# dog-qiuqiu/Yolo-FastestV2

Hardware: NVIDIA H100
Metric: images/sec 352x352 fwd+decode+NMS (higher is better)
Workload: dtype f32

## Files before the change

include/yfv2.h:

```cpp
#ifndef YFV2_H_
#define YFV2_H_

#include <stddef.h>
#include <stdint.h>

#ifdef __cplusplus
extern "C" {
#endif

#define YFV2_OK            0
#define YFV2_EINVAL       -1
#define YFV2_ECUDA        -2
#define YFV2_EUNSUPPORTED -3
#define YFV2_ENOMEM       -4

#define YFV2_ABI_VERSION   1

#if defined(__GNUC__)
#define YFV2_API __attribute__((visibility("default")))
#else
#define YFV2_API
#endif

#define YFV2_NUM_PARAMS    225
// ... 34 lines not shown
YFV2_API int yfv2_nms_workspace_bytes(int N, int M, int C, size_t* bytes);
YFV2_API int yfv2_nms(const float* dets, int N, int M, int C, float conf_thres, double iou_thres,
             const int* class_filter, int n_filter, int max_det, float max_wh,
             float* out, int* counts, int* kept_idx, void* workspace, void* stream);

YFV2_API int yfv2_decode_nms(const float* const preds[6], int N, int H, int W, int A, int C,
                    const double* anchors_host, float conf_thres, double iou_thres,
                    const int* class_filter, int n_filter, int max_det, float max_wh,
                    float* out, int* counts, int* kept_idx, void* workspace, void* stream);

YFV2_API int yfv2_batch_statistics(const float* dets, const int* counts, int N, int max_det, const float* targets, int nt,
                                   float iou_threshold, float* tp, void* stream);

YFV2_API int yfv2_aug_contrast_brightness(const uint8_t* img, uint8_t* out, const float* alpha, const float* beta, int N,
                                          long long bytes_per_image, void* stream);

typedef struct yfv2_frame {
    const uint8_t* data;
    int w, h;
    long long pitch;
} yfv2_frame;
YFV2_API int yfv2_resize_bgr_u8(const yfv2_frame* frames, int N, int H, int W, uint8_t* dst, void* stream);

typedef struct yfv2_yuv420_frame {
    const uint8_t* y;
    long long y_pitch;
    const uint8_t* u;
    const uint8_t* v;
    long long uv_pitch;
    int uv_step;
    int w, h;
} yfv2_yuv420_frame;
YFV2_API int yfv2_resize_yuv420_u8(const yfv2_yuv420_frame* frames, int N, int H, int W, uint8_t* dst, void* stream);

YFV2_API int yfv2_detect_u8_host(yfv2_plan* plan, const uint8_t* x_host, const void* packed,
                        const double* anchors_host, float conf_thres, double iou_thres, int max_det,
                        float* out_host, int* counts_host, void* workspace, void* stream);
YFV2_API size_t yfv2_detect_workspace_bytes(const yfv2_plan* plan, int max_det);

YFV2_API int yfv2_loss_workspace_bytes(int N, int H, int W, int A, int C, int nt, size_t* bytes);
YFV2_API int yfv2_compute_loss(const float* const preds[6], const float* targets, int nt, int N, int H, int W, int A, int C,
                               const double* anchors_host, float* losses, float* const dpreds[6], void* workspace,
                               void* stream);
YFV2_API int yfv2_loss_read_targets(const void* workspace, int level, int N, int H, int W, int A, int nt, int* count_host,
                                    int* idx, float* tbox, double* anch, int* tcls, void* stream);

YFV2_API int yfv2_op_conv1x1_fwd(const float* x, const float* w, const float* bias, float* y, int N, int K, int M, int HW, void* stream);
YFV2_API int yfv2_op_conv1x1_bwd(const float* x, const float* w, const float* dy, float* dx, float* dw, float* dbias, int N, int K, int M,
                                 int HW, void* stream);
YFV2_API int yfv2_op_dwconv_fwd(const float* x, const float* w, float* y, int N, int C, int H, int W, int ks, int stride, void* stream);
YFV2_API int yfv2_op_dwconv_bwd(const float* x, const float* w, const float* dy, float* dx, float* dw, int N, int C, int H, int W, int ks,
                                int stride, void* stream);
YFV2_API int yfv2_op_stem_fwd(const float* x, const float* w, float* y, int N, int M, int H, int W, void* stream);
YFV2_API int yfv2_op_stem_wgrad(const float* x, const float* dy, float* dw, int N, int M, int H, int W, void* stream);
YFV2_API int yfv2_op_bn_train_fwd(const float* x, const float* gamma, const float* beta, float* running_mean, float* running_var, float* y,
                                  float* save_mean, float* save_invstd, double* scratch, int N, int C, int HW, int relu, void* stream);
YFV2_API int yfv2_op_bn_train_bwd(const float* x, const float* y, const float* dy, const float* gamma, const float* save_mean,
                                  const float* save_invstd, float* dx, float* dgamma, float* dbeta, double* scratch, int N, int C, int HW,
                                  int relu, void* stream);
YFV2_API int yfv2_op_maxpool_fwd(const float* x, float* y, int* idx, int planes, int H, int W, void* stream);
YFV2_API int yfv2_op_maxpool_bwd(const float* dy, const int* idx, float* dx, int planes, int H, int W, void* stream);
YFV2_API int yfv2_op_upsample2_fwd(const float* x, float* y, int planes, int H, int W, void* stream);
YFV2_API int yfv2_op_upsample2_bwd(const float* dy, float* dx, int planes, int H, int W, void* stream);

typedef struct yfv2_trainer yfv2_trainer;
YFV2_API int yfv2_trainer_create(yfv2_trainer** out, int device, int N, int H, int W, int A, int C);
YFV2_API void yfv2_trainer_destroy(yfv2_trainer* t);
YFV2_API int yfv2_trainer_workspace_bytes(const yfv2_trainer* t, size_t* bytes);
YFV2_API int yfv2_trainer_grad_floats(const yfv2_trainer* t, long long* n);
YFV2_API int yfv2_trainer_param_offset(const yfv2_trainer* t, int index, long long* offset, long long* numel);
YFV2_API int yfv2_train_forward(yfv2_trainer* t, const float* x, const float* const* params, float* const* bn_running,
                                float* const preds[6], void* workspace, void* stream);
YFV2_API int yfv2_train_backward(yfv2_trainer* t, const float* x, const float* const* params, float* const preds[6],
                                 const float* const dpreds[6], float* grads_flat, int accumulate, void* workspace, void* stream);

YFV2_API const char* yfv2_plan_stage_name(const yfv2_plan* plan, int i);
YFV2_API int yfv2_plan_stage_group(const yfv2_plan* plan, int i);
YFV2_API int yfv2_forward_range(yfv2_plan* plan, const void* x, int is_u8, const void* packed, float* const preds[6],
                                void* workspace, int first, int last, void* stream);

YFV2_API int yfv2_debug_gather(const yfv2_plan* plan, const void* workspace, int which, float* out, int* dims4,
                               void* stream);

YFV2_API int yfv2_debug_pw_tc(const float* x, const float* w, float* out, float* pack_ws, int K, int N, int P,
                              void* stream);

YFV2_API int yfv2_debug_nms_profile(long long* dev_buf);

#ifdef __cplusplus
}
#endif
#endif
```

yolo-fastestv2_b200/csrc/k_net.cu:

```cuda
#include "common.cuh"
#include "tc.cuh"

namespace yfv2 {

namespace {
using namespace tc;

constexpr int kThreads = 256;
constexpr int kWarps = kThreads / 32;
constexpr int kMaxChain = 7;
constexpr size_t kChainBudget = 110 * 1024;
constexpr size_t kBandBudget = 110 * 1024;

__host__ __device__ constexpr int pw_smem_floats(int K, int NP) { return K * w_stride(NP) + 2 * NP; }

__device__ void load_pw(float* dst, const float* __restrict__ src, int K, int N, int NP) {
    const int S = w_stride(NP), Np = round4(N);
    for (int i = threadIdx.x; i < K * NP; i += blockDim.x) {
        const int k = i / NP, n = i - k * NP;
        dst[k * S + n] = n < N ? __ldg(src + k * Np + n) : 0.f;
    }
    for (int n = threadIdx.x; n < NP; n += blockDim.x) {
        dst[K * S + n] = n < N ? __ldg(src + K * Np + n) : 0.f;
        dst[K * S + NP + n] = n < N ? __ldg(src + K * Np + Np + n) : 0.f;
// ... 659 lines not shown

template <int K>
int dispatch_blk(int stride, BlkArgs& a, int N, cudaStream_t s) {
    return stride == 1 ? run_blk<K, 1>(a, N, s) : run_blk<K, 2>(a, N, s);
}

template <class Kern>
int run_whole_image(Kern kern, size_t bytes, BlkArgs& a, int N, cudaStream_t s) {
    a.R = a.Ho; a.bands = 1; a.items = N;
    if (int rc = smem_attr(kern, bytes)) return rc;
    int per_sm = 0;
    YFV2_CUDA(cudaOccupancyMaxActiveBlocksPerMultiprocessor(&per_sm, kern, kThreads, bytes));
    YFV2_CUDA(launch_k(kern, persistent_grid(N, per_sm > 0 ? per_sm : 1), kThreads, bytes, s, pdl_take(), a));
    YFV2_LAUNCH_CHECK();
    return YFV2_OK;
}

struct FpnArgs {
    Planes c3, c2, out;
    unsigned short t3[192], t2[96];
    const float* pw;
    int N, H, W, chunks;
};

template <int KIN>
__global__ void __launch_bounds__(kThreads)
fpn_kernel(const __grid_constant__ FpnArgs p) {
    pdl_trigger();
    constexpr int NT = 9, S = w_stride(72);
    extern __shared__ __align__(16) float smem[];
    load_pw(smem, p.pw, KIN, 72, 72);
    pdl_wait();
    __syncthreads();
    const int warp = threadIdx.x >> 5, lane = threadIdx.x & 31, g = lane >> 2, t = lane & 3;
    const int HW = p.H * p.W;
    for (int item = blockIdx.x; item < p.N * p.chunks; item += gridDim.x) {
        const int n = item / p.chunks, m0 = (item - n * p.chunks) * 16 * kWarps + 16 * warp;
        if (m0 >= HW) continue;
        int o3[2], o2[2], oo[2]; bool ok[2];
#pragma unroll
        for (int h = 0; h < 2; ++h) {
            const int m = m0 + g + 8 * h, y = m / p.W, x = m - y * p.W;
            ok[h] = m < HW;
            const int yy = ok[h] ? y : 0, xx = ok[h] ? x : 0;
            o3[h] = KIN == 192 ? p.c3.org + yy * p.c3.Ws + xx : p.c3.org + (yy >> 1) * p.c3.Ws + (xx >> 1);
            o2[h] = p.c2.org + yy * p.c2.Ws + xx;
            oo[h] = p.out.org + yy * p.out.Ws + xx;
        }
        const float* b3 = p.c3.base + (long long)n * p.c3.sN;
        const float* b2 = p.c2.base + (long long)n * p.c2.sN;
        float acc[NT][4];
        warp_gemm<KIN / 8, NT>(acc, smem, S, [&](int ks, float (&a)[4]) {
#pragma unroll
            for (int q = 0; q < 2; ++q) {
                const int k = 8 * ks + t + 4 * q;
                const float* pl = k < 192 ? b3 + (long long)p.t3[k] * p.c3.sC : b2 + (long long)p.t2[k - 192] * p.c2.sC;
#pragma unroll
                for (int h = 0; h < 2; ++h) a[2 * q + h] = pl[k < 192 ? o3[h] : o2[h]];
            }
        });
        float* ob = p.out.base + (long long)n * p.out.sN;
        const float* sc = smem + KIN * S;
#pragma unroll
        for (int h = 0; h < 2; ++h) {
            if (!ok[h]) continue;
#pragma unroll
            for (int nt = 0; nt < NT; ++nt)
#pragma unroll
                for (int e = 0; e < 2; ++e) {
                    const int col = 8 * nt + 2 * t + e;
                    ob[(long long)col * p.out.sC + oo[h]] = fmaxf(fmaf(acc[nt][2 * h + e], sc[col], sc[72 + col]), 0.f);
                }
        }
    }
}

struct HeadArgs {
    Planes in[2], out[2];
    const float* dw[2];
    const float* pw[2];
    float* dst[2][2];
    int split[2], rowsA[2], rowsB[2];
    int N, H, W, chunks;
};

constexpr int kHeadTile = 96;

template <int HALF>
__device__ __forceinline__ void head_body(const HeadArgs& p) {
    pdl_trigger();
    constexpr int NP = HALF == 0 ? 72 : HALF == 1 ? kHeadTile : 2 * kHeadTile;
    constexpr int NT = HALF == 0 ? 9 : HALF == 1 ? kHeadTile / 8 : kHeadTile / 16, S = w_stride(NP);
    extern __shared__ __align__(16) float smem[];
    float* sW = smem;
    float* sD = sW + pw_smem_floats(72, NP);
    const int br = blockIdx.y;
    const int tiles = HALF == 2 && br == 0 ? 2 : 1;
    if (HALF == 0) {
        load_pw(sW, p.pw[br], 72, 72, 72);
    } else {
        const float* F = p.pw[br];
        const int NF = HALF == 2 ? kHeadTile * tiles : NP;
        for (int i = threadIdx.x; i < 72 * NF; i += kThreads) {
            const int k = i / NF, nn = i - k * NF;
            sW[k * S + nn] = __ldg(F + nn * 72 + k);
        }
        for (int nn = threadIdx.x; nn < NF; nn += kThreads) { sW[72 * S + nn] = 1.f; sW[72 * S + NP + nn] = __ldg(F + NF * 72 + nn); }
    }
    load_floats(sD, p.dw[br], 72 * 28);
    pdl_wait();
    __syncthreads();
    const int warp = threadIdx.x >> 5, lane = threadIdx.x & 31, g = lane >> 2, t = lane & 3;
    const int HW = p.H * p.W;
    const Planes in = p.in[br];
    for (int item = blockIdx.x; item < p.N * p.chunks; item += gridDim.x) {
        const int n = item / p.chunks, m0 = (item - n * p.chunks) * 16 * kWarps + 16 * warp;
        if (m0 >= HW) continue;
        int off[2]; bool ok[2];
#pragma unroll
        for (int h = 0; h < 2; ++h) {
            const int m = m0 + g + 8 * h, y = m / p.W, x = m - y * p.W;
            ok[h] = m < HW;
            off[h] = ok[h] ? in.org + (y - 2) * in.Ws + x - 2 : in.org;
        }
        const float* ib = in.base + (long long)n * in.sN;
        auto load_a = [&](int ks, float (&a)[4]) {
#pragma unroll
            for (int q = 0; q < 2; ++q) {
                const int k = 8 * ks + t + 4 * q;
                const float* w = sD + 28 * k;
                const float* pk = ib + (long long)k * in.sC;
#pragma unroll
                for (int h = 0; h < 2; ++h) {
                    const float* tp = pk + off[h];
                    float v = 0.f;
#pragma unroll
                    for (int dy = 0; dy < 5; ++dy)
#pragma unroll
                        for (int dx = 0; dx < 5; ++dx) v = fmaf(tp[dy * in.Ws + dx], w[dy * 5 + dx], v);
                    a[2 * q + h] = ok[h] ? fmaxf(fmaf(v, w[25], w[26]), 0.f) : 0.f;
                }
            }
        };
        auto store = [&](const float (&acc)[NT][4], int c0) {
            const float* sc = sW + 72 * S;
#pragma unroll
            for (int h = 0; h < 2; ++h) {
                if (!ok[h]) continue;
                const int m = m0 + g + 8 * h;
#pragma unroll
                for (int nt = 0; nt < NT; ++nt)
#pragma unroll
                    for (int e = 0; e < 2; ++e) {
                        const int col = c0 + 8 * nt + 2 * t + e;
                        const float v = fmaf(acc[nt][2 * h + e], sc[col], sc[NP + col]);
                        if (HALF == 0) {
                            const Planes& o = p.out[br];
                            const int y = m / p.W, x = m - y * p.W;
                            o.base[(long long)n * o.sN + (long long)col * o.sC + o.org + y * o.Ws + x] = v;
                        } else if (col < p.split[br]) {
                            p.dst[br][0][((long long)n * p.rowsA[br] + col) * HW + m] = v;
                        } else if (col < p.split[br] + p.rowsB[br]) {
                            p.dst[br][1][((long long)n * p.rowsB[br] + col - p.split[br]) * HW + m] = v;
                        }
                    }
            }
        };
        if constexpr (HALF < 2) {
            float acc[NT][4];
            warp_gemm<9, NT>(acc, sW, S, load_a);
            store(acc, 0);
        } else {
            float af[9][4];
#pragma unroll
            for (int ks = 0; ks < 9; ++ks) load_a(ks, af[ks]);
#pragma unroll 1
            for (int c0 = 0; c0 < kHeadTile * tiles; c0 += 8 * NT) {
                float acc[NT][4];
                warp_gemm_regs<9, NT>(acc, sW + c0, S, af);
                store(acc, c0);
            }
        }
    }
}

template <int HALF>
__global__ void __launch_bounds__(kThreads)
head_kernel(const __grid_constant__ HeadArgs p) { head_body<HALF>(p); }

__global__ void __launch_bounds__(kThreads, 2)
head2_kernel(const __grid_constant__ HeadArgs p) { head_body<2>(p); }

template <int K, int NP>
__global__ void __launch_bounds__(kThreads)
pw_test_kernel(const float* __restrict__ x, const float* __restrict__ w, float* __restrict__ out, int N, int P) {
    constexpr int S = w_stride(NP);
    extern __shared__ __align__(16) float smem[];
    for (int i = threadIdx.x; i < K * NP; i += kThreads) {
        const int k = i / NP, nn = i - k * NP;
        smem[k * S + nn] = nn < N ? w[nn * K + k] : 0.f;
    }
    __syncthreads();
    const int warp = threadIdx.x >> 5, lane = threadIdx.x & 31, g = lane >> 2, t = lane & 3;
    const int m0 = (blockIdx.x * kWarps + warp) * 16;
    if (m0 >= P) return;
    float acc[NP / 8][4];
    warp_gemm<K / 8, NP / 8>(acc, smem, S, [&](int ks, float (&a)[4]) {
#pragma unroll
        for (int q = 0; q < 2; ++q)
#pragma unroll
            for (int h = 0; h < 2; ++h) {
                const int m = m0 + g + 8 * h;
                a[2 * q + h] = m < P ? x[(size_t)(8 * ks + t + 4 * q) * P + m] : 0.f;
            }
    });
#pragma unroll
    for (int h = 0; h < 2; ++h) {
        const int m = m0 + g + 8 * h;
        if (m >= P) continue;
#pragma unroll
        for (int nt = 0; nt < NP / 8; ++nt)
#pragma unroll
            for (int e = 0; e < 2; ++e) {
                const int col = 8 * nt + 2 * t + e;
                if (col < N) out[(size_t)col * P + m] = acc[nt][2 * h + e];
            }
    }
}

template <int K, int NP>
int run_pw_test(const float* x, const float* w, float* out, int N, int P, cudaStream_t s) {
    const size_t bytes = (size_t)K * w_stride(NP) * sizeof(float);
    if (int rc = smem_attr(pw_test_kernel<K, NP>, bytes)) return rc;
    pw_test_kernel<K, NP><<<(P + 16 * kWarps - 1) / (16 * kWarps), kThreads, bytes, s>>>(x, w, out, N, P);
    YFV2_LAUNCH_CHECK();
    return YFV2_OK;
}

}

bool blk_s1_chainable(int K, int H, int W) {
    const size_t bytes = blk_smem_bytes(K, 1, H, W);
    return bytes <= kChainBudget || (K == 96 && bytes <= kSmemCap);
}

int blk_launch_s1(int K, const Planes& P, int nblk, const ChanTab* tin, const ChanTab* tout, const float* const* w1,
                  const float* const* wdw, const float* const* w2, int N, cudaStream_t s) {
    if (nblk < 1 || nblk > kMaxChain || (nblk > 1 && !blk_s1_chainable(K, P.H, P.W))) {
        set_error("block: a chain of %d stride-1 blocks needs a whole %dx%d image per CTA", nblk, P.H, P.W);
        return YFV2_EINVAL;
    }
    BlkArgs a{};
    a.in = P; a.out = P;
    a.Hi = a.Ho = P.H; a.Wi = a.Wo = P.W;
    a.nblk = nblk;
    a.R = nblk > 1 ? P.H : blk_rows(K, 1, P.H, P.W, N);
    for (int j = 0; j < nblk; ++j) {
        a.pw1[j] = w1[j]; a.dw[j] = wdw[j]; a.pw2[j] = w2[j];
        for (int i = 0; i < K; ++i) { a.tin[j][i] = tin[j].c[i]; a.tout[j][i] = tout[j].c[i]; }
    }
    const size_t bytes = blk_smem_bytes(K, 1, P.H, P.W);
    if (nblk > 1 && bytes > kChainBudget) return run_whole_image(blk_chain_kernel<96>, bytes, a, N, s);
    switch (K) {
    case 24: return dispatch_blk<24>(1, a, N, s);
    case 48: return dispatch_blk<48>(1, a, N, s);
    case 96: return dispatch_blk<96>(1, a, N, s);
    }
    set_error("block: unsupported width %d", K);
    return YFV2_EUNSUPPORTED;
}

int blk_launch_s2(int K, const Planes& in, const Planes& out, const ChanTab& tin, const ChanTab& tout, const float* wdwp, const float* wp,
                  const float* w1, const float* wdwm, const float* w2, int N, cudaStream_t s) {
    BlkArgs a{};
    a.in = in; a.out = out;
    a.Hi = in.H; a.Wi = in.W; a.Ho = out.H; a.Wo = out.W;
    a.nblk = 1;
    a.pw1[0] = w1; a.dw[0] = wdwm; a.pw2[0] = w2; a.dwp = wdwp; a.pwp = wp;
    for (int i = 0; i < K; ++i) { a.tin[0][i] = tin.c[i]; a.tout[0][i] = tout.c[i]; a.tmain[i] = tout.c[K + i]; }
    if (blk_s2_whole_image(K, out.H, out.W, in.W))
        return run_whole_image(blk_s2_image_kernel<96>, blk_s2_image_smem_bytes(K, out.H, in.W), a, N, s);
    a.R = blk_rows(K, 2, out.H, in.W, N);
    if (blk_s2_walk_fits(K, in)) return K == 24 ? run_blk_walk<24>(a, N, s) : run_blk_walk<48>(a, N, s);
    switch (K) {
    case 24: return dispatch_blk<24>(2, a, N, s);
    case 48: return dispatch_blk<48>(2, a, N, s);
    case 96: return dispatch_blk<96>(2, a, N, s);
    }
    set_error("block: unsupported width %d", K);
    return YFV2_EUNSUPPORTED;
}

int fpn_launch(int which, const Planes& c3, const ChanTab& t3, const Planes& c2, const ChanTab& t2, const Planes& out, const float* pw,
               int N, cudaStream_t s) {
    FpnArgs a{};
    a.c3 = c3; a.c2 = c2; a.out = out; a.pw = pw;
    for (int i = 0; i < 192; ++i) a.t3[i] = t3.c[i];
    for (int i = 0; i < 96; ++i) a.t2[i] = t2.c[i];
    a.N = N; a.H = out.H; a.W = out.W;
    a.chunks = (out.H * out.W + 16 * kWarps - 1) / (16 * kWarps);
    auto run = [&](auto kern, int kin) -> int {
        const size_t bytes = (size_t)pw_smem_floats(kin, 72) * sizeof(float);
        if (int rc = smem_attr(kern, bytes)) return rc;
        YFV2_CUDA(launch_k(kern, persistent_grid((long long)N * a.chunks, 2), kThreads, bytes, s, pdl_take(), a));
        YFV2_LAUNCH_CHECK();
        return YFV2_OK;
    };
    return which == 1 ? run(fpn_kernel<192>, 192) : run(fpn_kernel<288>, 288);
}

int heads_launch(int half, const Planes& sIn, const Planes& tcls, const Planes& treg, const float* const wdw[2], const float* const wpw[2],
                 float* reg, float* obj, float* cls, int A, int C, int N, cudaStream_t s) {
    HeadArgs a{};
    for (int b = 0; b < 2; ++b) { a.dw[b] = wdw[b]; a.pw[b] = wpw[b]; }
    a.out[0] = tcls; a.out[1] = treg;
    if (half == 0) { a.in[0] = sIn; a.in[1] = sIn; }
    else { a.in[0] = tcls; a.in[1] = treg; }
    a.dst[0][0] = obj; a.dst[0][1] = cls; a.split[0] = A; a.rowsA[0] = A; a.rowsB[0] = C;
    a.dst[1][0] = reg; a.dst[1][1] = reg; a.split[1] = 4 * A; a.rowsA[1] = 4 * A; a.rowsB[1] = 0;
    a.N = N; a.H = sIn.H; a.W = sIn.W;
    a.chunks = (sIn.H * sIn.W + 16 * kWarps - 1) / (16 * kWarps);
    auto run = [&](auto kern, int np) -> int {
        const size_t bytes = ((size_t)pw_smem_floats(72, np) + 72 * 28) * sizeof(float);
        if (int rc = smem_attr(kern, bytes)) return rc;
        cudaLaunchConfig_t cfg{};
        cfg.gridDim = dim3((unsigned)persistent_grid((long long)N * a.chunks, 1), 2);
        cfg.blockDim = dim3(kThreads); cfg.dynamicSmemBytes = bytes; cfg.stream = s;
        cudaLaunchAttribute at[1];
        at[0].id = cudaLaunchAttributeProgrammaticStreamSerialization;
        at[0].val.programmaticStreamSerializationAllowed = 1;
        cfg.attrs = at; cfg.numAttrs = pdl_take() ? 1 : 0;
        YFV2_CUDA(cudaLaunchKernelEx(&cfg, kern, a));
        YFV2_LAUNCH_CHECK();
        return YFV2_OK;
    };
    if (half == 0) return run(head_kernel<0>, 72);
    if (A + C <= kHeadTile) return run(head_kernel<1>, kHeadTile);
    if (A + C <= 2 * kHeadTile && 4 * A <= kHeadTile) return run(head2_kernel, 2 * kHeadTile);
    set_error("heads: anchors+classes = %d exceeds two %d-column output tiles", A + C, kHeadTile);
    return YFV2_EUNSUPPORTED;
}
static_assert((pw_smem_floats(72, 2 * kHeadTile) + 72 * 28) * sizeof(float) <= kSmemCap, "two head tiles must fit in shared memory");

}

using namespace yfv2;

extern "C" int yfv2_debug_pw_tc(const float* x, const float* w, float* out, float* pack_ws, int K, int N, int P, void* stream) {
    (void)pack_ws;
    if (!x || !w || !out || P <= 0) { set_error("debug_pw_tc: bad argument"); return YFV2_EINVAL; }
    cudaStream_t s = (cudaStream_t)stream;
    if (K == 24 && N == 24) return run_pw_test<24, 24>(x, w, out, N, P, s);
    if (K == 48 && N == 48) return run_pw_test<48, 48>(x, w, out, N, P, s);
    if (K == 96 && N == 96) return run_pw_test<96, 96>(x, w, out, N, P, s);
    if (K == 72 && N == 72) return run_pw_test<72, 72>(x, w, out, N, P, s);
    if (K == 72 && N == 83) return run_pw_test<72, 88>(x, w, out, N, P, s);
    set_error("debug_pw_tc: unsupported K=%d N=%d", K, N);
    return YFV2_EUNSUPPORTED;
}
```

yolo-fastestv2_b200/csrc/plan.cu:

```cuda
#include <stdarg.h>
#include <string.h>

#include <new>
#include <vector>

#include <stdlib.h>

#include "common.cuh"

namespace yfv2 {

bool blk_s1_chainable(int K, int H, int W);

static thread_local char g_err[512] = "";

void set_error(const char* fmt, ...) {
    va_list ap;
    va_start(ap, fmt);
    vsnprintf(g_err, sizeof(g_err), fmt, ap);
    va_end(ap);
}

static thread_local bool g_pdl_next = false;
static thread_local bool g_pdl_call = true;
// ... 339 lines not shown
    pack_dw_kernel<<<(Cn * KK + 255) / 256, 256, 0, s>>>(w, Cn, KK, R, g, b, m, v, pack);
    YFV2_LAUNCH_CHECK();
    return YFV2_OK;
}

#define TRY(x) do { int rc__ = (x); if (rc__) return rc__; } while (0)

}

extern "C" int yfv2_pack_weights(yfv2_plan* p, const float* const* params, const float* const* bn_running, void* packed,
                                 void* stream) {
    if (!p || !params || !bn_running || !packed) { set_error("pack_weights: null argument"); return YFV2_EINVAL; }
    cudaStream_t s = (cudaStream_t)stream;
    float* pk = (float*)packed;
    YFV2_CUDA(cudaMemsetAsync(pk, 0, p->pk_floats * sizeof(float), s));
    Cursor cur{params, bn_running};
    TRY(pack_pw(cur, true, false, 24, 27, pk + p->pk_stem, 24, 0, s));
    for (int b = 0; b < kNumBlocks; ++b) {
        const int K = p->blk_K[b];
        float* d = pk + p->pk_block[b];
        const int pwn = pw_pack_floats(K, K), dwn = dw3_pack_floats(K);
        if (p->blk_stride[b] == 2) {
            TRY(pack_pw(cur, true, false, K, K, d + dwn + pwn, K, 0, s));
            TRY(pack_dw(cur, K, 3, d + dwn + 2 * pwn, s));
            TRY(pack_pw(cur, true, false, K, K, d + 2 * dwn + 2 * pwn, K, 0, s));
            TRY(pack_dw(cur, K, 3, d, s));
            TRY(pack_pw(cur, true, false, K, K, d + dwn, K, 0, s));
        } else {
            TRY(pack_pw(cur, true, false, K, K, d, K, 0, s));
            TRY(pack_dw(cur, K, 3, d + pwn, s));
            TRY(pack_pw(cur, true, false, K, K, d + pwn + dwn, K, 0, s));
        }
    }
    TRY(pack_pw(cur, true, false, kFpnDepth, 288, pk + p->pk_fpn2, kFpnDepth, 0, s));
    TRY(pack_pw(cur, true, false, kFpnDepth, 192, pk + p->pk_fpn3, kFpnDepth, 0, s));
    const int head_order[4] = {0, 1, 3, 2};
    struct Pw2 { const float *w, *g, *b, *m, *v; } pw2[4];
    for (int i = 0; i < 4; ++i) {
        float* d = pk + p->pk_head[head_order[i]];
        const int dwn = dw5_pack_floats(kFpnDepth), pwn = pw_pack_floats(kFpnDepth, kFpnDepth);
        const int hi_ = head_order[i];
        TRY(pack_dw(cur, kFpnDepth, 5, d, s));
        TRY(pack_pw(cur, true, false, kFpnDepth, kFpnDepth, d + dwn, kFpnDepth, 0, s));
        TRY(pack_dw(cur, kFpnDepth, 5, d + dwn + pwn, s));
        pw2[hi_] = Pw2{cur.params[cur.p], cur.params[cur.p + 1], cur.params[cur.p + 2], cur.bn[2 * cur.b], cur.bn[2 * cur.b + 1]};
        TRY(pack_pw(cur, true, false, kFpnDepth, kFpnDepth, d + 2 * dwn + pwn, kFpnDepth, 0, s));
    }
    const float* wo[3] = {cur.params[cur.p], cur.params[cur.p + 2], cur.params[cur.p + 4]};
    const float* bo[3] = {cur.params[cur.p + 1], cur.params[cur.p + 3], cur.params[cur.p + 5]};
    TRY(pack_pw(cur, false, true, 4 * p->A, kFpnDepth, pk + p->pk_out_reg, round4(4 * p->A), 0, s));
    const int Moc = round4(p->A + p->C);
    TRY(pack_pw(cur, false, true, p->A, kFpnDepth, pk + p->pk_out_oc, Moc, 0, s));
    TRY(pack_pw(cur, false, true, p->C, kFpnDepth, pk + p->pk_out_oc, Moc, p->A, s));
    for (int h = 0; h < 4; ++h) {
        const Pw2& q = pw2[h];
        float* Fw = pk + p->pk_foldw[h];
        float* Fb = Fw + (size_t)p->fold_rows[h] * kFpnDepth;
        const int K = kFpnDepth;
        auto fold = [&](int which, int Mo, int n_off) -> int {
            if (!wo[which] || !bo[which]) { set_error("pack_weights: null output-layer tensor"); return YFV2_EINVAL; }
            fold_head_kernel<<<(Mo * K + 255) / 256, 256, 0, s>>>(wo[which], bo[which], Mo, q.w, q.g, q.b, q.m, q.v, K, n_off, Fw, Fb);
            YFV2_LAUNCH_CHECK();
            return YFV2_OK;
        };
        if (h & 1) { TRY(fold(0, 4 * p->A, 0)); }
        else { TRY(fold(1, p->A, 0)); TRY(fold(2, p->C, p->A)); }
    }
    if (cur.p != YFV2_NUM_PARAMS || cur.b != YFV2_NUM_BN) {
        set_error("pack_weights: internal walk consumed %d params / %d BN layers", cur.p, cur.b);
        return YFV2_EINVAL;
    }
    return YFV2_OK;
}

namespace yfv2 {
int blk_launch_s1(int K, const Planes& P, int nblk, const ChanTab* tin, const ChanTab* tout, const float* const* w1,
                  const float* const* wdw, const float* const* w2, int N, cudaStream_t s);
int blk_launch_s2(int K, const Planes& in, const Planes& out, const ChanTab& tin, const ChanTab& tout, const float* wdwp, const float* wp,
                  const float* w1, const float* wdwm, const float* w2, int N, cudaStream_t s);
int fpn_launch(int which, const Planes& c3, const ChanTab& t3, const Planes& c2, const ChanTab& t2, const Planes& out, const float* pw,
               int N, cudaStream_t s);
int heads_launch(int half, const Planes& sIn, const Planes& tcls, const Planes& treg, const float* const wdw[2], const float* const wpw[2],
                 float* reg, float* obj, float* cls, int A, int C, int N, cudaStream_t s);
}

namespace {
int forward_impl(yfv2_plan* p, const void* x, int is_u8, const void* packed, float* const preds[6], void* workspace,
                 int first, int last, cudaStream_t s) {
    if (!p || !x || !packed || !preds || !workspace) { set_error("forward: null argument"); return YFV2_EINVAL; }
    for (int i = 0; i < 6; ++i) if (!preds[i]) { set_error("forward: null output %d", i); return YFV2_EINVAL; }
    if (last < 0) last = p->n_stages;
    if (first < 0 || last > p->n_stages || first > last) { set_error("forward: bad stage range [%d,%d)", first, last); return YFV2_EINVAL; }
    float* ws = (float*)workspace;
    const float* pk = (const float*)packed;
    pdl_reset();
    if (p->ws_zeroed != workspace) {
        YFV2_CUDA(cudaMemsetAsync(workspace, 0, p->ws_floats * sizeof(float), s));
        p->ws_zeroed = workspace;
    }
    struct { Planes c3, c2, s3, s2; ChanTab t3, t2; } f;
    f.c3 = pool_planes(p, ws, 3); f.t3 = p->c3;
    f.c2 = pool_planes(p, ws, 2); f.t2 = p->c2;
    f.s3 = flat_planes(p, ws, p->off_s3, 3);
    f.s2 = flat_planes(p, ws, p->off_s2, 2);
    for (int si = first; si < last; ++si) {
        const yfv2_plan::Stage& st = p->stages[si];
        const int b = st.a;
        switch (st.kind) {
        case 0: {
            StemArgs a{x, is_u8, p->N, p->H, p->W, pool_planes(p, ws, 0), pk + p->pk_stem};
            TRY(launch_stem(a, s));
        } break;
        case 15: {
            const int lv = st.a, half = st.b;
            const Planes sIn = lv ? f.s3 : f.s2;
            const Planes t_cls = flat_planes(p, ws, p->off_t[2 * lv], 2 + lv);
            const Planes t_reg = flat_planes(p, ws, p->off_t[2 * lv + 1], 2 + lv);
            const float* w_cls = pk + p->pk_head[2 * lv];
            const float* w_reg = pk + p->pk_head[2 * lv + 1];
            const size_t dwn = dw5_pack_floats(kFpnDepth), half_off = (size_t)half * (dwn + pw_pack_floats(kFpnDepth, kFpnDepth));
            const float* wdw[2] = {w_cls + half_off, w_reg + half_off};
            const float* wpw[2] = {half ? pk + p->pk_foldw[2 * lv] : w_cls + dwn, half ? pk + p->pk_foldw[2 * lv + 1] : w_reg + dwn};
            TRY(heads_launch(half, sIn, t_cls, t_reg, wdw, wpw, preds[3 * lv], preds[3 * lv + 1], preds[3 * lv + 2], p->A, p->C, p->N, s));
        } break;
        case 10: {
            const int K = p->blk_K[b];
            int nb = 1;
            while (si + nb < last && p->stages[si + nb].group == st.group) ++nb;
            const float *w1[7], *w2[7], *wd[7];
            for (int j = 0; j < nb; ++j) {
                const float* d = pk + p->pk_block[b + j];
                const int pwn = pw_pack_floats(K, K);
                w1[j] = d; wd[j] = d + pwn; w2[j] = d + pwn + dw3_pack_floats(K);
            }
            TRY(blk_launch_s1(K, pool_planes(p, ws, p->blk_res[b]), nb, &p->tin[b], &p->tout[b], w1, wd, w2, p->N, s));
            si += nb - 1;
        } break;
        case 11: {
            const int K = p->blk_K[b];
            const float* d = pk + p->pk_block[b];
            const int dwn = dw3_pack_floats(K), pwn = pw_pack_floats(K, K);
            TRY(blk_launch_s2(K, pool_planes(p, ws, p->blk_res[b] - 1), pool_planes(p, ws, p->blk_res[b]), p->tin[b], p->tout[b],
                              d, d + dwn, d + dwn + pwn, d + dwn + 2 * pwn, d + 2 * dwn + 2 * pwn, p->N, s));
        } break;
        case 14: {
            if (st.a == 1) { TRY(fpn_launch(1, f.c3, f.t3, f.c2, f.t2, f.s3, pk + p->pk_fpn3, p->N, s)); }
            else { TRY(fpn_launch(2, f.c3, f.t3, f.c2, f.t2, f.s2, pk + p->pk_fpn2, p->N, s)); }
        } break;
        default: set_error("forward: unknown stage kind %d", st.kind); return YFV2_EINVAL;
        }
    }
    return YFV2_OK;
}
}

extern "C" int yfv2_forward_range(yfv2_plan* p, const void* x, int is_u8, const void* packed, float* const preds[6],
                                  void* workspace, int first, int last, void* stream) {
    return forward_impl(p, x, is_u8, packed, preds, workspace, first, last, (cudaStream_t)stream);
}

extern "C" int yfv2_forward(yfv2_plan* p, const float* x, const void* packed, float* const preds[6], void* workspace,
                            void* stream) {
    return forward_impl(p, x, 0, packed, preds, workspace, 0, -1, (cudaStream_t)stream);
}

extern "C" int yfv2_forward_u8(yfv2_plan* p, const uint8_t* x, const void* packed, float* const preds[6], void* workspace,
                               void* stream) {
    return forward_impl(p, x, 1, packed, preds, workspace, 0, -1, (cudaStream_t)stream);
}

namespace {
struct DetectLayout {
    size_t off_x, off_pred[6], off_out, off_counts, total;
};
DetectLayout detect_layout(const yfv2_plan* p, int max_det) {
    DetectLayout L;
    size_t off = align_up(p->ws_floats * sizeof(float), 256);
    L.off_x = off; off += align_up((size_t)p->N * 3 * p->H * p->W, 256);
    for (int lv = 0; lv < 2; ++lv) {
        const size_t hw = (size_t)p->h[2 + lv] * p->w[2 + lv];
        const int ch[3] = {4 * p->A, p->A, p->C};
        for (int k = 0; k < 3; ++k) { L.off_pred[3 * lv + k] = off; off += align_up((size_t)p->N * ch[k] * hw * sizeof(float), 256); }
    }
    L.off_out = off; off += align_up((size_t)p->N * max_det * 6 * sizeof(float), 256);
    L.off_counts = off; off += align_up((size_t)p->N * sizeof(int), 256);
    L.total = off;
    return L;
}
}

extern "C" size_t yfv2_detect_workspace_bytes(const yfv2_plan* p, int max_det) {
    if (!p || max_det <= 0) return 0;
    return detect_layout(p, max_det).total;
}

extern "C" int yfv2_detect_u8_host(yfv2_plan* p, const uint8_t* x_host, const void* packed, const double* anchors_host,
                                   float conf_thres, double iou_thres, int max_det, float* out_host, int* counts_host,
                                   void* workspace, void* stream) {
    if (!p || !x_host || !packed || !anchors_host || !out_host || !counts_host || !workspace || max_det <= 0) {
        set_error("detect_u8_host: null argument");
        return YFV2_EINVAL;
    }
    cudaStream_t s = (cudaStream_t)stream;
    const DetectLayout L = detect_layout(p, max_det);
    unsigned char* ws = (unsigned char*)workspace;
    uint8_t* x_dev = ws + L.off_x;
    float* preds[6];
    for (int i = 0; i < 6; ++i) preds[i] = (float*)(ws + L.off_pred[i]);
    float* out_dev = (float*)(ws + L.off_out);
    int* counts_dev = (int*)(ws + L.off_counts);
    YFV2_CUDA(cudaMemcpyAsync(x_dev, x_host, (size_t)p->N * 3 * p->H * p->W, cudaMemcpyHostToDevice, s));
    struct PdlOff { PdlOff() { g_pdl_call = false; } ~PdlOff() { g_pdl_call = true; } } pdl_off_guard;
    TRY(forward_impl(p, x_dev, 1, packed, preds, ws, 0, -1, s));
    TRY(yfv2_decode_nms(preds, p->N, p->H, p->W, p->A, p->C, anchors_host, conf_thres, iou_thres, nullptr, 0, max_det,
                        4096.0f, out_dev, counts_dev, nullptr, nullptr, stream));
    YFV2_CUDA(cudaMemcpyAsync(out_host, out_dev, (size_t)p->N * max_det * 6 * sizeof(float), cudaMemcpyDeviceToHost, s));
    YFV2_CUDA(cudaMemcpyAsync(counts_host, counts_dev, (size_t)p->N * sizeof(int), cudaMemcpyDeviceToHost, s));
    return YFV2_OK;
}

extern "C" int yfv2_debug_gather(const yfv2_plan* p, const void* workspace, int which, float* out, int* dims4, void* stream) {
    if (!p || !workspace || !dims4) { set_error("debug_gather: null argument"); return YFV2_EINVAL; }
    float* ws = (float*)workspace;
    Planes P; ChanTab tab; int Cn;
    for (int i = 0; i < kMaxCh; ++i) tab.c[i] = (unsigned short)i;
    if (which == 0) { P = pool_planes(p, ws, 0); Cn = 24; }
    else if (which >= 1 && which <= kNumBlocks) { const int b = which - 1; P = pool_planes(p, ws, p->blk_res[b]); Cn = 2 * p->blk_K[b]; tab = p->logical[b]; }
    else if (which == 17) { P = flat_planes(p, ws, p->off_s2, 2); Cn = kFpnDepth; }
    else if (which == 18) { P = flat_planes(p, ws, p->off_s3, 3); Cn = kFpnDepth; }
    else if (which >= 19 && which <= 22) { const int i = which - 19; P = flat_planes(p, ws, p->off_t[i], i < 2 ? 2 : 3); Cn = kFpnDepth; }
    else { set_error("debug_gather: unknown tensor id %d", which); return YFV2_EINVAL; }
    dims4[0] = p->N; dims4[1] = Cn; dims4[2] = P.H; dims4[3] = P.W;
    if (!out) return YFV2_OK;
    const long long total = (long long)p->N * Cn * P.H * P.W;
    gather_kernel<<<(unsigned)((total + 255) / 256), 256, 0, (cudaStream_t)stream>>>(P, tab, Cn, out, total);
    YFV2_LAUNCH_CHECK();
    return YFV2_OK;
}
```

yolo-fastestv2_b200/yfv2_engine.py:

```python
import ctypes
import os
import threading

import torch

_HERE = os.path.dirname(os.path.abspath(__file__))
_LIB_PATH = os.path.join(_HERE, "libyfv2.so")
_lib = None
_lock = threading.Lock()

MAX_DET = 300
MAX_WH = 4096.0

_c_float_p = ctypes.POINTER(ctypes.c_float)
_c_void_pp = ctypes.POINTER(ctypes.c_void_p)


class Frame(ctypes.Structure):
    _fields_ = [("data", ctypes.c_void_p), ("w", ctypes.c_int), ("h", ctypes.c_int), ("pitch", ctypes.c_longlong)]


class Yuv420Frame(ctypes.Structure):
    _fields_ = [("y", ctypes.c_void_p), ("y_pitch", ctypes.c_longlong), ("u", ctypes.c_void_p), ("v", ctypes.c_void_p),
                ("uv_pitch", ctypes.c_longlong), ("uv_step", ctypes.c_int), ("w", ctypes.c_int), ("h", ctypes.c_int)]


PROTOTYPES = {
    "yfv2_abi_version": (ctypes.c_int, []),
    "yfv2_last_error": (ctypes.c_char_p, []),
    "yfv2_plan_create": (ctypes.c_int, [_c_void_pp, ctypes.c_int, ctypes.c_int, ctypes.c_int, ctypes.c_int,
                                        ctypes.c_int, ctypes.c_int, ctypes.c_int]),
    "yfv2_plan_destroy": (ctypes.c_int, [ctypes.c_void_p]),
    "yfv2_plan_workspace_bytes": (ctypes.c_int, [ctypes.c_void_p, ctypes.POINTER(ctypes.c_size_t)]),
    "yfv2_plan_invalidate_workspace": (ctypes.c_int, [ctypes.c_void_p]),
    "yfv2_plan_packed_bytes": (ctypes.c_int, [ctypes.c_void_p, ctypes.POINTER(ctypes.c_size_t)]),
    "yfv2_plan_forward_launches": (ctypes.c_int, [ctypes.c_void_p, ctypes.POINTER(ctypes.c_int)]),
    "yfv2_pack_weights": (ctypes.c_int, [ctypes.c_void_p, _c_void_pp, _c_void_pp, ctypes.c_void_p, ctypes.c_void_p]),
    "yfv2_forward": (ctypes.c_int, [ctypes.c_void_p, ctypes.c_void_p, ctypes.c_void_p, _c_void_pp, ctypes.c_void_p,
                                    ctypes.c_void_p]),
    "yfv2_forward_u8": (ctypes.c_int, [ctypes.c_void_p, ctypes.c_void_p, ctypes.c_void_p, _c_void_pp, ctypes.c_void_p,
                                       ctypes.c_void_p]),
    "yfv2_decode": (ctypes.c_int, [_c_void_pp, ctypes.c_int, ctypes.c_int, ctypes.c_int, ctypes.c_int, ctypes.c_int,
                                   ctypes.POINTER(ctypes.c_double), ctypes.c_void_p, ctypes.c_void_p]),
    "yfv2_export_heads": (ctypes.c_int, [_c_void_pp, ctypes.c_int, ctypes.c_int, ctypes.c_int, ctypes.c_int, ctypes.c_int,
                                         ctypes.c_void_p, ctypes.c_void_p, ctypes.c_void_p]),
    "yfv2_nms_workspace_bytes": (ctypes.c_int, [ctypes.c_int, ctypes.c_int, ctypes.c_int, ctypes.POINTER(ctypes.c_size_t)]),
    "yfv2_nms": (ctypes.c_int, [ctypes.c_void_p, ctypes.c_int, ctypes.c_int, ctypes.c_int, ctypes.c_float, ctypes.c_double,
                                ctypes.c_void_p, ctypes.c_int, ctypes.c_int, ctypes.c_float, ctypes.c_void_p,
                                ctypes.c_void_p, ctypes.c_void_p, ctypes.c_void_p, ctypes.c_void_p]),
    "yfv2_decode_nms": (ctypes.c_int, [_c_void_pp, ctypes.c_int, ctypes.c_int, ctypes.c_int, ctypes.c_int, ctypes.c_int,
                                       ctypes.POINTER(ctypes.c_double), ctypes.c_float, ctypes.c_double, ctypes.c_void_p,
                                       ctypes.c_int, ctypes.c_int, ctypes.c_float, ctypes.c_void_p, ctypes.c_void_p,
                                       ctypes.c_void_p, ctypes.c_void_p, ctypes.c_void_p]),
    "yfv2_batch_statistics": (ctypes.c_int, [ctypes.c_void_p, ctypes.c_void_p, ctypes.c_int, ctypes.c_int, ctypes.c_void_p,
                                             ctypes.c_int, ctypes.c_float, ctypes.c_void_p, ctypes.c_void_p]),
    "yfv2_aug_contrast_brightness": (ctypes.c_int, [ctypes.c_void_p] * 4 + [ctypes.c_int, ctypes.c_longlong, ctypes.c_void_p]),
    "yfv2_resize_bgr_u8": (ctypes.c_int, [ctypes.POINTER(Frame), ctypes.c_int, ctypes.c_int, ctypes.c_int, ctypes.c_void_p,
                                          ctypes.c_void_p]),
    "yfv2_resize_yuv420_u8": (ctypes.c_int, [ctypes.POINTER(Yuv420Frame), ctypes.c_int, ctypes.c_int, ctypes.c_int, ctypes.c_void_p,
                                             ctypes.c_void_p]),
    "yfv2_detect_u8_host": (ctypes.c_int, [ctypes.c_void_p, ctypes.c_void_p, ctypes.c_void_p,
                                           ctypes.POINTER(ctypes.c_double), ctypes.c_float, ctypes.c_double, ctypes.c_int,
                                           ctypes.c_void_p, ctypes.c_void_p, ctypes.c_void_p, ctypes.c_void_p]),
    "yfv2_detect_workspace_bytes": (ctypes.c_size_t, [ctypes.c_void_p, ctypes.c_int]),
    "yfv2_loss_workspace_bytes": (ctypes.c_int, [ctypes.c_int] * 6 + [ctypes.POINTER(ctypes.c_size_t)]),
    "yfv2_compute_loss": (ctypes.c_int, [_c_void_pp, ctypes.c_void_p, ctypes.c_int, ctypes.c_int, ctypes.c_int, ctypes.c_int,
                                         ctypes.c_int, ctypes.c_int, ctypes.POINTER(ctypes.c_double), ctypes.c_void_p, _c_void_pp,
                                         ctypes.c_void_p, ctypes.c_void_p]),
    "yfv2_loss_read_targets": (ctypes.c_int, [ctypes.c_void_p, ctypes.c_int, ctypes.c_int, ctypes.c_int, ctypes.c_int, ctypes.c_int,
                                              ctypes.c_int, ctypes.POINTER(ctypes.c_int), ctypes.c_void_p, ctypes.c_void_p,
                                              ctypes.c_void_p, ctypes.c_void_p, ctypes.c_void_p]),
    "yfv2_op_conv1x1_fwd": (ctypes.c_int, [ctypes.c_void_p] * 4 + [ctypes.c_int] * 4 + [ctypes.c_void_p]),
    "yfv2_op_conv1x1_bwd": (ctypes.c_int, [ctypes.c_void_p] * 6 + [ctypes.c_int] * 4 + [ctypes.c_void_p]),
    "yfv2_op_dwconv_fwd": (ctypes.c_int, [ctypes.c_void_p] * 3 + [ctypes.c_int] * 6 + [ctypes.c_void_p]),
    "yfv2_op_dwconv_bwd": (ctypes.c_int, [ctypes.c_void_p] * 5 + [ctypes.c_int] * 6 + [ctypes.c_void_p]),
    "yfv2_op_stem_fwd": (ctypes.c_int, [ctypes.c_void_p] * 3 + [ctypes.c_int] * 4 + [ctypes.c_void_p]),
    "yfv2_op_stem_wgrad": (ctypes.c_int, [ctypes.c_void_p] * 3 + [ctypes.c_int] * 4 + [ctypes.c_void_p]),
    "yfv2_op_bn_train_fwd": (ctypes.c_int, [ctypes.c_void_p] * 9 + [ctypes.c_int] * 4 + [ctypes.c_void_p]),
    "yfv2_op_bn_train_bwd": (ctypes.c_int, [ctypes.c_void_p] * 10 + [ctypes.c_int] * 4 + [ctypes.c_void_p]),
    "yfv2_op_maxpool_fwd": (ctypes.c_int, [ctypes.c_void_p] * 3 + [ctypes.c_int] * 3 + [ctypes.c_void_p]),
    "yfv2_op_maxpool_bwd": (ctypes.c_int, [ctypes.c_void_p] * 3 + [ctypes.c_int] * 3 + [ctypes.c_void_p]),
    "yfv2_op_upsample2_fwd": (ctypes.c_int, [ctypes.c_void_p] * 2 + [ctypes.c_int] * 3 + [ctypes.c_void_p]),
    "yfv2_op_upsample2_bwd": (ctypes.c_int, [ctypes.c_void_p] * 2 + [ctypes.c_int] * 3 + [ctypes.c_void_p]),
    "yfv2_trainer_create": (ctypes.c_int, [_c_void_pp] + [ctypes.c_int] * 6),
    "yfv2_trainer_destroy": (None, [ctypes.c_void_p]),
    "yfv2_trainer_workspace_bytes": (ctypes.c_int, [ctypes.c_void_p, ctypes.POINTER(ctypes.c_size_t)]),
    "yfv2_trainer_grad_floats": (ctypes.c_int, [ctypes.c_void_p, ctypes.POINTER(ctypes.c_longlong)]),
    "yfv2_trainer_param_offset": (ctypes.c_int, [ctypes.c_void_p, ctypes.c_int, ctypes.POINTER(ctypes.c_longlong), ctypes.POINTER(ctypes.c_longlong)]),
    "yfv2_train_forward": (ctypes.c_int, [ctypes.c_void_p, ctypes.c_void_p, _c_void_pp, _c_void_pp, _c_void_pp, ctypes.c_void_p, ctypes.c_void_p]),
    "yfv2_train_backward": (ctypes.c_int, [ctypes.c_void_p, ctypes.c_void_p, _c_void_pp, _c_void_pp, _c_void_pp, ctypes.c_void_p, ctypes.c_int,
                                           ctypes.c_void_p, ctypes.c_void_p]),
    "yfv2_plan_stage_name": (ctypes.c_char_p, [ctypes.c_void_p, ctypes.c_int]),
    "yfv2_plan_stage_group": (ctypes.c_int, [ctypes.c_void_p, ctypes.c_int]),
    "yfv2_forward_range": (ctypes.c_int, [ctypes.c_void_p, ctypes.c_void_p, ctypes.c_int, ctypes.c_void_p, _c_void_pp,
                                          ctypes.c_void_p, ctypes.c_int, ctypes.c_int, ctypes.c_void_p]),
    "yfv2_debug_pw_tc": (ctypes.c_int, [ctypes.c_void_p, ctypes.c_void_p, ctypes.c_void_p, ctypes.c_void_p, ctypes.c_int,
                                        ctypes.c_int, ctypes.c_int, ctypes.c_void_p]),
    "yfv2_debug_gather": (ctypes.c_int, [ctypes.c_void_p, ctypes.c_void_p, ctypes.c_int, ctypes.c_void_p,
                                         ctypes.POINTER(ctypes.c_int), ctypes.c_void_p]),
    "yfv2_debug_nms_profile": (ctypes.c_int, [ctypes.c_void_p]),
    "yfv2_ncnn_post": (ctypes.c_int, [ctypes.c_void_p, ctypes.c_void_p, ctypes.c_int, ctypes.c_int, ctypes.c_int, ctypes.c_int, ctypes.c_int,
                                      ctypes.POINTER(ctypes.c_float), ctypes.c_float, ctypes.c_float, ctypes.c_float, ctypes.c_float,
                                      ctypes.c_int, ctypes.c_void_p, ctypes.c_void_p, ctypes.c_void_p, ctypes.c_void_p, ctypes.c_void_p]),
}


def lib():
    global _lib
    if _lib is None:
        with _lock:
            if _lib is None:
                if not os.path.exists(_LIB_PATH):
                    raise RuntimeError("libyfv2.so is missing (%s): build it with "
                                       "`python yolo-fastestv2_b200/build.py` or __graft_entry__.build()" % _LIB_PATH)
                L = ctypes.CDLL(_LIB_PATH)
                for name, (res, args) in PROTOTYPES.items():
                    fn = getattr(L, name)
                    fn.restype, fn.argtypes = res, args
                _lib = L
    return _lib


class Yfv2Error(RuntimeError):
    pass


def _check(rc, what):
    if rc != 0:
        raise Yfv2Error("%s failed (%d): %s" % (what, rc, lib().yfv2_last_error().decode("utf-8", "replace")))


def _stream(device):
    return ctypes.c_void_p(torch.cuda.current_stream(device).cuda_stream)


def _ptr_array(tensors):
    arr = (ctypes.c_void_p * len(tensors))()
    for i, t in enumerate(tensors):
        arr[i] = t.data_ptr()
    return arr


def _require_cuda(t, name):
    if not isinstance(t, torch.Tensor) or not t.is_cuda:
        raise Yfv2Error("%s must be a CUDA tensor: this implementation has no CPU path" % name)


class Trainer:

    def __init__(self, device, N, H, W, A, C):
        L = lib()
        self.device = torch.device(device)
        if self.device.type != "cuda":
            raise Yfv2Error("trainers exist on CUDA devices only")
        self.N, self.H, self.W, self.A, self.C = N, H, W, A, C
        self._h = ctypes.c_void_p()
        with torch.cuda.device(self.device):
            _check(L.yfv2_trainer_create(ctypes.byref(self._h), self.device.index or 0, N, H, W, A, C), "trainer_create")
        nb = ctypes.c_size_t()
        _check(L.yfv2_trainer_workspace_bytes(self._h, ctypes.byref(nb)), "trainer_workspace_bytes")
        self.workspace = torch.empty(nb.value, dtype=torch.uint8, device=self.device)
        n = ctypes.c_longlong()
        _check(L.yfv2_trainer_grad_floats(self._h, ctypes.byref(n)), "trainer_grad_floats")
        self.grad_floats = n.value
        self.param_offsets = []
        off, num = ctypes.c_longlong(), ctypes.c_longlong()
        for i in range(225):
            _check(L.yfv2_trainer_param_offset(self._h, i, ctypes.byref(off), ctypes.byref(num)), "trainer_param_offset")
            self.param_offsets.append((off.value, num.value))
        self.generation = 0
        self.x_static = torch.empty((N, 3, H, W), dtype=torch.float32, device=self.device)
        self.preds_static = self.alloc_preds()
        self.dpreds_static = [torch.empty_like(p) for p in self.preds_static]
        self.flat_static = torch.empty(self.grad_floats, dtype=torch.float32, device=self.device)

    def __del__(self):
        try:
            if getattr(self, "_h", None) is not None and self._h.value:
                lib().yfv2_trainer_destroy(self._h)
                self._h = ctypes.c_void_p()
        except Exception:
            pass

# ... 517 lines not shown
```

Baseline: 66960.

## Stage head input windows into shared memory via multi-slot cp.async pipeline

The detection head kernel now copies each chunk's input row window for 8 channels at a time into a three-slot shared-memory ring with cp.async. It overlaps those copies with the 5x5 depthwise and tensor-core pointwise compute, instead of reading taps directly from global memory. A host-side check picks the window stride and enables staging only when the alignment and shared-memory budget allow it, and launch bounds are raised to request two blocks per SM. The per-k-step waits and block barriers, plus the larger shared-memory footprint, could cost synchronization overhead and occupancy. A debug entry point reports whether the staged path is chosen.

```diff
diff --git a/include/yfv2.h b/include/yfv2.h
--- a/include/yfv2.h
+++ b/include/yfv2.h
@@ -140,6 +140,8 @@
 YFV2_API int yfv2_debug_gather(const yfv2_plan* plan, const void* workspace, int which, float* out, int* dims4,
                                void* stream);
 
+YFV2_API int yfv2_debug_heads_staged(const yfv2_plan* plan, const void* workspace, int which);
+
 YFV2_API int yfv2_debug_pw_tc(const float* x, const float* w, float* out, float* pack_ws, int K, int N, int P,
                               void* stream);
 
diff --git a/yolo-fastestv2_b200/csrc/k_net.cu b/yolo-fastestv2_b200/csrc/k_net.cu
--- a/yolo-fastestv2_b200/csrc/k_net.cu
+++ b/yolo-fastestv2_b200/csrc/k_net.cu
@@ -765,9 +765,26 @@
     float* dst[2][2];
     int split[2], rowsA[2], rowsB[2];
     int N, H, W, chunks;
+    int CS;
 };
 
 constexpr int kHeadTile = 96;
+constexpr int kHeadSlots = 3;
+constexpr size_t kHeadBudget = 113 * 1024;
+
+__host__ __device__ constexpr int head_win_rows(int H, int W) {
+    return ((W - 1 + 16 * kWarps - 1) / W + 1 < H ? (W - 1 + 16 * kWarps - 1) / W + 1 : H) + 4;
+}
+__host__ constexpr size_t head_weight_bytes(int NP) { return ((size_t)pw_smem_floats(72, NP) + 72 * 28) * sizeof(float); }
+
+__device__ __forceinline__ float dw5_bn_relu(const float* tp, int ld, const float* w) {
+    float v = 0.f;
+#pragma unroll
+    for (int dy = 0; dy < 5; ++dy)
+#pragma unroll
+        for (int dx = 0; dx < 5; ++dx) v = fmaf(tp[dy * ld + dx], w[dy * 5 + dx], v);
+    return fmaxf(fmaf(v, w[25], w[26]), 0.f);
+}
 
 template <int HALF>
 __device__ __forceinline__ void head_body(const HeadArgs& p) {
@@ -777,6 +794,7 @@
     extern __shared__ __align__(16) float smem[];
     float* sW = smem;
     float* sD = sW + pw_smem_floats(72, NP);
+    float* X = sD + 72 * 28;
     const int br = blockIdx.y;
     const int tiles = HALF == 2 && br == 0 ? 2 : 1;
     if (HALF == 0) {
@@ -792,22 +810,59 @@
     }
     load_floats(sD, p.dw[br], 72 * 28);
     pdl_wait();
+    const int warp = threadIdx.x >> 5, lane = threadIdx.x & 31, g = lane >> 2, t = lane & 3;
+    const int HW = p.H * p.W, items = p.N * p.chunks, CS = p.CS;
+    const Planes& in = p.in[br];
+    auto chunk_rows = [&](int chunk, int& y0, int& len) {
+        const int m = chunk * 16 * kWarps;
+        y0 = m / p.W;
+        len = ((min(HW, m + 16 * kWarps) - 1) / p.W - y0 + 5) * in.Ws;
+    };
+    auto stage = [&](int j) {
+        const int item = blockIdx.x + j / 9 * gridDim.x;
+        if (item < items) {
+            const int n = item / p.chunks;
+            int y0, len;
+            chunk_rows(item - n * p.chunks, y0, len);
+            const float* src = in.base + (long long)n * in.sN + (long long)(8 * (j % 9) + warp) * in.sC + (long long)y0 * in.Ws;
+            float* dst = X + (j % kHeadSlots * 8 + warp) * CS;
+            for (int o = 4 * lane; o < len; o += 128) cp16(dst + o, src + o);
+        }
+        cp_async_commit();
+    };
+    if (CS) {
+        for (int j = 0; j < kHeadSlots - 1; ++j) stage(j);
+    }
     __syncthreads();
-    const int warp = threadIdx.x >> 5, lane = threadIdx.x & 31, g = lane >> 2, t = lane & 3;
-    const int HW = p.H * p.W;
-    const Planes in = p.in[br];
-    for (int item = blockIdx.x; item < p.N * p.chunks; item += gridDim.x) {
-        const int n = item / p.chunks, m0 = (item - n * p.chunks) * 16 * kWarps + 16 * warp;
-        if (m0 >= HW) continue;
+    for (int item = blockIdx.x, j0 = 0; item < items; item += gridDim.x, j0 += 9) {
+        const int n = item / p.chunks, chunk = item - n * p.chunks, m0 = chunk * 16 * kWarps + 16 * warp;
+        if (!CS && m0 >= HW) continue;
+        int y0, len;
+        chunk_rows(chunk, y0, len);
         int off[2]; bool ok[2];
 #pragma unroll
         for (int h = 0; h < 2; ++h) {
             const int m = m0 + g + 8 * h, y = m / p.W, x = m - y * p.W;
             ok[h] = m < HW;
-            off[h] = ok[h] ? in.org + (y - 2) * in.Ws + x - 2 : in.org;
-        }
+            off[h] = CS ? (ok[h] ? (y - y0) * in.Ws + x : 0) : ok[h] ? in.org + (y - 2) * in.Ws + x - 2 : in.org;
+        }
+        auto load_staged = [&](int ks, float (&a)[4]) {
+            cp_async_wait<kHeadSlots - 2>();
+            __syncthreads();
+            stage(j0 + ks + kHeadSlots - 1);
+            const float* slot = X + (j0 + ks) % kHeadSlots * 8 * CS;
+#pragma unroll
+            for (int q = 0; q < 2; ++q) {
+                const float* w = sD + 28 * (8 * ks + t + 4 * q);
+#pragma unroll
+                for (int h = 0; h < 2; ++h) {
+                    const float v = dw5_bn_relu(slot + (t + 4 * q) * CS + off[h], in.Ws, w);
+                    a[2 * q + h] = ok[h] ? v : 0.f;
+                }
+            }
+        };
         const float* ib = in.base + (long long)n * in.sN;
-        auto load_a = [&](int ks, float (&a)[4]) {
+        auto load_planes = [&](int ks, float (&a)[4]) {
 #pragma unroll
             for (int q = 0; q < 2; ++q) {
                 const int k = 8 * ks + t + 4 * q;
@@ -815,13 +870,8 @@
                 const float* pk = ib + (long long)k * in.sC;
 #pragma unroll
                 for (int h = 0; h < 2; ++h) {
-                    const float* tp = pk + off[h];
-                    float v = 0.f;
-#pragma unroll
-                    for (int dy = 0; dy < 5; ++dy)
-#pragma unroll
-                        for (int dx = 0; dx < 5; ++dx) v = fmaf(tp[dy * in.Ws + dx], w[dy * 5 + dx], v);
-                    a[2 * q + h] = ok[h] ? fmaxf(fmaf(v, w[25], w[26]), 0.f) : 0.f;
+                    const float v = dw5_bn_relu(pk + off[h], in.Ws, w);
+                    a[2 * q + h] = ok[h] ? v : 0.f;
                 }
             }
         };
@@ -849,26 +899,30 @@
                     }
             }
         };
-        if constexpr (HALF < 2) {
-            float acc[NT][4];
-            warp_gemm<9, NT>(acc, sW, S, load_a);
-            store(acc, 0);
-        } else {
-            float af[9][4];
-#pragma unroll
-            for (int ks = 0; ks < 9; ++ks) load_a(ks, af[ks]);
+        auto contract = [&](auto&& load_a) {
+            if constexpr (HALF < 2) {
+                float acc[NT][4];
+                warp_gemm<9, NT>(acc, sW, S, load_a);
+                store(acc, 0);
+            } else {
+                float af[9][4];
+#pragma unroll
+                for (int ks = 0; ks < 9; ++ks) load_a(ks, af[ks]);
 #pragma unroll 1
-            for (int c0 = 0; c0 < kHeadTile * tiles; c0 += 8 * NT) {
-                float acc[NT][4];
-                warp_gemm_regs<9, NT>(acc, sW + c0, S, af);
-                store(acc, c0);
-            }
-        }
+                for (int c0 = 0; c0 < kHeadTile * tiles; c0 += 8 * NT) {
+                    float acc[NT][4];
+                    warp_gemm_regs<9, NT>(acc, sW + c0, S, af);
+                    store(acc, c0);
+                }
+            }
+        };
+        if (CS) contract(load_staged);
+        else contract(load_planes);
     }
 }
 
 template <int HALF>
-__global__ void __launch_bounds__(kThreads)
+__global__ void __launch_bounds__(kThreads, 2)
 head_kernel(const __grid_constant__ HeadArgs p) { head_body<HALF>(p); }
 
 __global__ void __launch_bounds__(kThreads, 2)
@@ -992,9 +1046,26 @@
     return which == 1 ? run(fpn_kernel<192>, 192) : run(fpn_kernel<288>, 288);
 }
 
+int head_columns(int half, int A, int C) {
+    if (half == 0) return 72;
+    if (A + C <= kHeadTile) return kHeadTile;
+    if (A + C <= 2 * kHeadTile && 4 * A <= kHeadTile) return 2 * kHeadTile;
+    return 0;
+}
+
+int heads_window_stride(int half, const Planes& sIn, const Planes& tcls, const Planes& treg, int A, int C) {
+    const int np = head_columns(half, A, C);
+    const Planes* in[2] = {half ? &tcls : &sIn, half ? &treg : &sIn};
+    for (const Planes* q : in)
+        if (q->pad != 2 || ((uintptr_t)q->base & 15) || q->Ws % 4 || q->sC % 4 || q->sN % 4 || q->Ws != in[0]->Ws) return 0;
+    const int cs = walk::ring_stride(head_win_rows(in[0]->H, in[0]->W) * in[0]->Ws);
+    return np && head_weight_bytes(np) + (size_t)kHeadSlots * 8 * cs * sizeof(float) <= kHeadBudget ? cs : 0;
+}
+
 int heads_launch(int half, const Planes& sIn, const Planes& tcls, const Planes& treg, const float* const wdw[2], const float* const wpw[2],
                  float* reg, float* obj, float* cls, int A, int C, int N, cudaStream_t s) {
     HeadArgs a{};
+    a.CS = heads_window_stride(half, sIn, tcls, treg, A, C);
     for (int b = 0; b < 2; ++b) { a.dw[b] = wdw[b]; a.pw[b] = wpw[b]; }
     a.out[0] = tcls; a.out[1] = treg;
     if (half == 0) { a.in[0] = sIn; a.in[1] = sIn; }
@@ -1004,7 +1075,7 @@
     a.N = N; a.H = sIn.H; a.W = sIn.W;
     a.chunks = (sIn.H * sIn.W + 16 * kWarps - 1) / (16 * kWarps);
     auto run = [&](auto kern, int np) -> int {
-        const size_t bytes = ((size_t)pw_smem_floats(72, np) + 72 * 28) * sizeof(float);
+        const size_t bytes = head_weight_bytes(np) + (size_t)kHeadSlots * 8 * a.CS * sizeof(float);
         if (int rc = smem_attr(kern, bytes)) return rc;
         cudaLaunchConfig_t cfg{};
         cfg.gridDim = dim3((unsigned)persistent_grid((long long)N * a.chunks, 1), 2);
@@ -1017,13 +1088,15 @@
         YFV2_LAUNCH_CHECK();
         return YFV2_OK;
     };
-    if (half == 0) return run(head_kernel<0>, 72);
-    if (A + C <= kHeadTile) return run(head_kernel<1>, kHeadTile);
-    if (A + C <= 2 * kHeadTile && 4 * A <= kHeadTile) return run(head2_kernel, 2 * kHeadTile);
+    switch (head_columns(half, A, C)) {
+    case 72: return run(head_kernel<0>, 72);
+    case kHeadTile: return run(head_kernel<1>, kHeadTile);
+    case 2 * kHeadTile: return run(head2_kernel, 2 * kHeadTile);
+    }
     set_error("heads: anchors+classes = %d exceeds two %d-column output tiles", A + C, kHeadTile);
     return YFV2_EUNSUPPORTED;
 }
-static_assert((pw_smem_floats(72, 2 * kHeadTile) + 72 * 28) * sizeof(float) <= kSmemCap, "two head tiles must fit in shared memory");
+static_assert(head_weight_bytes(2 * kHeadTile) <= kSmemCap, "two head tiles must fit in shared memory");
 
 }
 
diff --git a/yolo-fastestv2_b200/csrc/plan.cu b/yolo-fastestv2_b200/csrc/plan.cu
--- a/yolo-fastestv2_b200/csrc/plan.cu
+++ b/yolo-fastestv2_b200/csrc/plan.cu
@@ -445,6 +445,7 @@
                int N, cudaStream_t s);
 int heads_launch(int half, const Planes& sIn, const Planes& tcls, const Planes& treg, const float* const wdw[2], const float* const wpw[2],
                  float* reg, float* obj, float* cls, int A, int C, int N, cudaStream_t s);
+int heads_window_stride(int half, const Planes& sIn, const Planes& tcls, const Planes& treg, int A, int C);
 }
 
 namespace {
@@ -600,3 +601,13 @@
     YFV2_LAUNCH_CHECK();
     return YFV2_OK;
 }
+
+extern "C" int yfv2_debug_heads_staged(const yfv2_plan* p, const void* workspace, int which) {
+    if (!p || !workspace || which < 0 || which > 3) { set_error("debug_heads_staged: bad argument"); return YFV2_EINVAL; }
+    float* ws = (float*)workspace;
+    const int lv = which / 2, half = which % 2;
+    const Planes sIn = flat_planes(p, ws, lv ? p->off_s3 : p->off_s2, 2 + lv);
+    const Planes t_cls = flat_planes(p, ws, p->off_t[2 * lv], 2 + lv);
+    const Planes t_reg = flat_planes(p, ws, p->off_t[2 * lv + 1], 2 + lv);
+    return heads_window_stride(half, sIn, t_cls, t_reg, p->A, p->C) > 0 ? 1 : 0;
+}
diff --git a/yolo-fastestv2_b200/yfv2_engine.py b/yolo-fastestv2_b200/yfv2_engine.py
--- a/yolo-fastestv2_b200/yfv2_engine.py
+++ b/yolo-fastestv2_b200/yfv2_engine.py
@@ -99,6 +99,7 @@
     "yfv2_debug_gather": (ctypes.c_int, [ctypes.c_void_p, ctypes.c_void_p, ctypes.c_int, ctypes.c_void_p,
                                          ctypes.POINTER(ctypes.c_int), ctypes.c_void_p]),
     "yfv2_debug_nms_profile": (ctypes.c_int, [ctypes.c_void_p]),
+    "yfv2_debug_heads_staged": (ctypes.c_int, [ctypes.c_void_p, ctypes.c_void_p, ctypes.c_int]),
     "yfv2_ncnn_post": (ctypes.c_int, [ctypes.c_void_p, ctypes.c_void_p, ctypes.c_int, ctypes.c_int, ctypes.c_int, ctypes.c_int, ctypes.c_int,
                                       ctypes.POINTER(ctypes.c_float), ctypes.c_float, ctypes.c_float, ctypes.c_float, ctypes.c_float,
                                       ctypes.c_int, ctypes.c_void_p, ctypes.c_void_p, ctypes.c_void_p, ctypes.c_void_p, ctypes.c_void_p]),
```

Result: faster. 69030 (median of 6 runs) (+3.1%).
